# SensorsINI/v2e

Hardware: AMD Instinct MI355X
Metric: Mevents/s (EventEmulator.generate_events, 346x260, 10x slowdown) (higher is better)
Workload: dtype f64

## Files before the change

v2e_amd/csrc/emu.hip:

```cpp
#include "common.h"
#include "../../include/v2e_detmath.h"

#include <cstdarg>
#include <cstdlib>
#include <chrono>
#include <vector>

namespace {

constexpr int BLOCK = 256;
constexpr int WAVE = 64;
constexpr int RING = 64;
constexpr int SCAN_BLOCKS = 64;
constexpr int STAMP_LAUNCHES = 128;

constexpr uint32_t CNT_MASK = 0x00FFFFFFu;
constexpr uint32_t CNT_NEG = 1u << 24;
constexpr uint32_t CNT_SHOT_ON = 1u << 25;
constexpr uint32_t CNT_SHOT_OFF = 1u << 26;

struct FrameCtl {
    double t_prev, t_frame;
    double dt_over_tau;
    double shot_base;
// ... 1438 lines not shown
            V2E_HIP(hipHostGetDevicePointer((void **)&h->fr_ev_host_dev, h->fr_ev_host, 0));
            h->fr_ev_cap = want;
        }
        k_frame_rows_to_host<<<(unsigned)std::min<uint64_t>(v2e_cdiv((int64_t)n, 256), 4096), 256, 0, s>>>(
            (const float4 *)events_dev, rec, (float4 *)h->fr_ev_host_dev, nullptr, 0ull, n, nullptr);
        V2E_HIP(hipGetLastError());
        V2E_HIP(hipStreamSynchronize(s));
        *events_host = h->fr_ev_host;
        return 0;
    }
    if (user_rows) {
        if (n > est) {
            k_frame_rows_to_host<<<(unsigned)std::min<uint64_t>(v2e_cdiv((int64_t)(n - est), 256), 4096), 256, 0, s>>>(
                (const float4 *)events_dev, rec, (float4 *)user_rows_dev, nullptr, est, n - est, nullptr);
            V2E_HIP(hipGetLastError());
            V2E_HIP(hipStreamSynchronize(s));
        }
        if (n > 0) *events_host = user_rows;
        return 0;
    }
    if (n > est) {
        if (n > h->fr_ev_cap) {
            float *grown = nullptr;
            const uint64_t want = std::max<uint64_t>(2 * n, 1u << 16);
            V2E_HIP(hipHostMalloc((void **)&grown, sizeof(float) * 4 * want, hipHostMallocMapped));
            memcpy(grown, h->fr_ev_host, sizeof(float) * 4 * est);
            V2E_HIP(hipHostFree(h->fr_ev_host));
            h->fr_ev_host = grown; h->fr_ev_cap = want;
            V2E_HIP(hipHostGetDevicePointer((void **)&h->fr_ev_host_dev, h->fr_ev_host, 0));
        }
        k_frame_rows_to_host<<<(unsigned)std::min<uint64_t>(v2e_cdiv((int64_t)(n - est), 256), 4096), 256, 0, s>>>(
            (const float4 *)events_dev, rec, (float4 *)h->fr_ev_host_dev, nullptr, est, n - est, nullptr);
        V2E_HIP(hipGetLastError());
        V2E_HIP(hipStreamSynchronize(s));
    }
    if (n > 0) *events_host = h->fr_ev_host;
    return 0;
}

int v2e_emu_frame_host_rows(v2e_emu *h, float *pinned_rows, uint64_t cap_rows)
{
    V2E_REQUIRE(h, "null");
    h->fr_user_rows = h->fr_user_rows_dev = nullptr; h->fr_user_cap = 0;
    if (!pinned_rows || cap_rows == 0) return 0;
    V2E_HIP(hipSetDevice(h->device));
    void *dev = nullptr;
    V2E_HIP(hipHostGetDevicePointer(&dev, pinned_rows, 0));
    h->fr_user_rows = pinned_rows; h->fr_user_rows_dev = (float *)dev; h->fr_user_cap = cap_rows;
    return 0;
}

static int enqueue_run(v2e_emu *h, const v2e_emu_params *p, const KArgs &a, const void *frames, int dtype, int n_frames,
                       float *events, uint64_t cap, v2e_frame_rec *recs, hipStream_t s, hipEvent_t *evs = nullptr)
{
#define V2E_MARK(i) do { if (evs) V2E_HIP(hipEventRecord(evs[(i)], s)); } while (0)
    const RunScratch &r = h->cur();
    const size_t esz = dtype == V2E_DT_U8 ? 1 : (dtype == V2E_DT_F32 ? 4 : 8);
    V2E_HIP(zero_async(recs, sizeof(v2e_frame_rec) * (size_t)n_frames * h->n_clips, s));
    dim3 gridw(v2e_cdiv((int64_t)h->nwaves * WAVE, BLOCK), h->n_clips);
    for (int f = 0; f < n_frames; ++f) {
        const void *fr = (const char *)frames + (size_t)f * h->n_clips * h->npx * esz;
        const FrameCtl *ctl = r.run_ctl + (size_t)f * h->n_clips;
        v2e_frame_rec *rec = recs + (size_t)f * h->n_clips;
        const v2e_frame_rec *rec_prev = f > 0 ? rec - h->n_clips : nullptr;
        V2E_MARK(4 * f + 0);
        if (h->cs_sur) {
            dim3 gridp(v2e_cdiv(h->npx, BLOCK), h->n_clips);
            DISPATCH_FT(dtype, {
                if (p->f64_state) k_cs_lp<double, FT><<<gridp, BLOCK, 0, s>>>(a, (const FT *)fr, ctl, (double *)h->csr_lp);
                else k_cs_lp<float, FT><<<gridp, BLOCK, 0, s>>>(a, (const FT *)fr, ctl, (float *)h->csr_lp);
            });
            int rcs = v2e_csdvs_enqueue_frame(h->csr_lp, const_cast<void *>(h->cs_sur), h->csr_scratch, h->H, h->W, p->f64_state,
                                              h->csr_ap[f], h->csr_ah[f], h->csr_steps[f], h->csr_thr, h->csr_slots, h->csr_steps_dev + f, s);
            if (rcs) return rcs;
        }
        int rc = launch_count(h, a, p->f64_state, fr, dtype, ctl, r.run_fidx, (uint32_t)f, nullptr, nullptr, rec, s);
        if (rc) return rc;
        V2E_MARK(4 * f + 1);
        k_rank<<<gridw, BLOCK, 0, s>>>(a, ctl, rec, nullptr, 0);
        V2E_MARK(4 * f + 2);
        k_scan<<<dim3(SCAN_BLOCKS, h->n_clips), BLOCK, 0, s>>>(a, rec);
        V2E_MARK(4 * f + 3);
        if (p->f64_state) k_emit<double><<<gridw, BLOCK, 0, s>>>(a, ctl, rec, rec_prev, nullptr, r.run_fidx, (uint32_t)f, nullptr, 0, (float4 *)events, cap);
        else k_emit<float><<<gridw, BLOCK, 0, s>>>(a, ctl, rec, rec_prev, nullptr, r.run_fidx, (uint32_t)f, nullptr, 0, (float4 *)events, cap);
    }
    V2E_MARK(4 * n_frames);
#undef V2E_MARK
    V2E_HIP(hipGetLastError());
    return 0;
}


enum { ST_MAIN = 0, ST_AHEAD = 1, ST_SIDE = 2, ST_TAB = 3, ST_SIDE2 = 4, ST_COUNT = 5 };
enum { EV_FORK = 0, EV_JOIN = 1, EV_AHEAD = 2, EV_CHAIN = 3, EV_TAB = 4 };

struct Sched {
    v2e_emu *h;
    hipStream_t st[ST_COUNT];

    hipEvent_t real_event(int kind, int idx) const
    {
        switch (kind) {
        case EV_FORK: return h->ev_fork[idx];
        case EV_JOIN: return h->ev_join[idx];
        case EV_AHEAD: return h->ev_ahead[idx];
        case EV_CHAIN: return h->ev_chain[idx];
        default: return h->ev_tab[idx];
        }
    }
    int kernel(int s, const void *fn, dim3 grid, dim3 block, size_t lds, void **args)
    {
        V2E_HIP(hipLaunchKernel(fn, grid, block, args, lds, st[s]));
        return 0;
    }
    int zero4(int s, void *const ptr[4], const size_t bytes[4])
    {
        ZeroRanges z;
        unsigned long long tot = 0;
        for (int r = 0; r < 4; ++r) { z.p[r] = (uint32_t *)ptr[r]; z.n[r] = ptr[r] ? (bytes[r] + 3) / 4 : 0; tot += z.n[r]; }
        if (tot == 0) return 0;
        void *args[] = {(void *)&z};
        return kernel(s, (const void *)k_zero_ranges, dim3((unsigned)((tot + 255) / 256)), dim3(256), 0, args);
    }
    int record(int kind, int idx, int s)
    {
        V2E_HIP(hipEventRecord(real_event(kind, idx), st[s]));
        return 0;
    }
    int wait(int s, int kind, int idx)
    {
        V2E_HIP(hipStreamWaitEvent(st[s], real_event(kind, idx), 0));
        return 0;
    }
};

static int chain_egroups(const v2e_emu *h) { return (h->npx + GROUP_PX - 1) / GROUP_PX; }
static bool chain_small_grid(const v2e_emu *h) { return (long long)h->ngroups * h->n_clips <= 2ll * h->n_cu; }

static int chain_ring_batches(v2e_emu *h, bool pipelined)
{
    if (h->ch_ring_pref == 0) h->ch_ring_pref = (pipelined && chain_small_grid(h) && h->n_clips == 1) ? 5 : 3;
    return h->ch_ring_pref;
}

static bool chain_fused_records(const v2e_emu *h, int dtype, int nD)
{
    if (dtype != V2E_DT_U8) return true;
    if ((size_t)nD * 64 * h->n_clips * h->npx_pad * sizeof(uint2) >= (1ull << 32)) return true;
    const char *fe = getenv("V2E_AMD_CHAIN_FUSED");
    const int fused_env = fe ? atoi(fe) : -1;
    return fused_env >= 0 ? fused_env != 0 : !chain_small_grid(h);
}

static size_t chain_dyn_lds(bool fused) { return fused ? 0 : (size_t)CHAIN_SUB * BLOCK * sizeof(uint2); }

static const void *chain_fn(bool f64, int dtype, bool fused, bool allon = false)
{
    if (allon && f64 && dtype == V2E_DT_U8)
        return fused ? (const void *)k_chain<double, uint8_t, true, true> : (const void *)k_chain<double, uint8_t, false, true>;
    if (!fused) return f64 ? (const void *)k_chain<double, uint8_t, false> : (const void *)k_chain<float, uint8_t, false>;
    switch (dtype) {
    case V2E_DT_U8: return f64 ? (const void *)k_chain<double, uint8_t, true> : (const void *)k_chain<float, uint8_t, true>;
    case V2E_DT_F32: return f64 ? (const void *)k_chain<double, float, true> : (const void *)k_chain<float, float, true>;
    default: return f64 ? (const void *)k_chain<double, double, true> : (const void *)k_chain<float, double, true>;
    }
}

static int chain_blocks_per_cu(v2e_emu *h, bool f64, int dtype, bool fused, bool allon = false)
{
    allon = allon && f64 && dtype == V2E_DT_U8;
    const int key = (f64 ? 1 : 0) | ((dtype & 3) << 1) | (fused ? 8 : 0) | (allon ? 16 : 0);
    if (h->occ_cache[key] >= 0) return h->occ_cache[key];
    int per_cu = 0;
    if (hipOccupancyMaxActiveBlocksPerMultiprocessor(&per_cu, chain_fn(f64, dtype, fused, allon), BLOCK, chain_dyn_lds(fused)) != hipSuccess) per_cu = 0;
    if (per_cu > 2) per_cu = std::min(per_cu - 1, 6);
    h->occ_cache[key] = per_cu;
    return per_cu;
}

static int chain_frames_per_launch(const v2e_emu *h, bool has_refr, int flags, int max_blocks)
{
    int K = !has_refr ? CHAIN_K_MAX : (chain_small_grid(h) ? 32 : 8);
    if (const char *ev = getenv("V2E_AMD_CHAIN_K")) { const int v = atoi(ev); if (v >= 1 && v <= CHAIN_K_MAX) K = v; }
    if (has_refr && ((flags & V2E_RUN_ONE_FRAME_PER_LAUNCH) || h->ngroups > max_blocks)) K = 1;
    return K;
}

struct ChainLaunch { int f0, nf, pf0, pnf, wait_join, wait_ahead, ahead_next, emit_batch; };
static std::vector<ChainLaunch> chain_plan(int n_frames, int K, int E, int nD, bool has_refr, bool fused)
{
    const int m = E / K;
    const int nB = (n_frames + K - 1) / K;
    const int nL = has_refr ? nB + 1 : nB;
    const int nEB = (n_frames + E - 1) / E;
    std::vector<ChainLaunch> plan;
    for (int L = 0; L < nL; ++L) {
        ChainLaunch c;
        const bool tail = L >= nB;
        c.f0 = tail ? n_frames : L * K;
        c.nf = tail ? 0 : std::min((L + 1) * K, n_frames) - L * K;
        c.pf0 = (L - 1) * K;
        c.pnf = (has_refr && L > 0) ? std::min(L * K, n_frames) - (L - 1) * K : 0;
        const bool first = !tail && L % m == 0;
        c.wait_join = (first && L / m >= nD) ? L / m - nD : -1;
        c.wait_ahead = (first && !fused) ? L / m : -1;
        c.ahead_next = (first && !fused && L / m + 2 < nEB) ? L / m + 2 : -1;
        const int fin = has_refr ? L - 1 : L;
        c.emit_batch = (fin >= 0 && ((fin + 1) % m == 0 || fin == nB - 1)) ? fin / m : -1;
        plan.push_back(c);
    }
    return plan;
}

static bool emit_pull(size_t table_bytes)
{
    if (const char *e = getenv("V2E_AMD_EMIT_PULL")) { if (atoi(e) == 0) return false; }
    size_t budget = (size_t)24 << 30;
    if (const char *e = getenv("V2E_AMD_PULL_BUDGET_MB")) { const long long v = atoll(e); if (v >= 0) budget = (size_t)v << 20; }
    size_t free_b = 0, total_b = 0;
    if (hipMemGetInfo(&free_b, &total_b) != hipSuccess) return false;
    return table_bytes <= free_b / 4 && table_bytes <= budget;
}

static int chain_alloc(v2e_emu *h, const v2e_emu_params *p, int dtype, int n_frames, int flags, bool pipelined)
{
    const bool has_refr = p->refractory_period_s > 0;
    const int nD = chain_ring_batches(h, pipelined);
    const bool fused = chain_fused_records(h, dtype, nD);
    const int inst = (p->f64_state ? 1 : 0) | ((dtype & 3) << 1) | (fused ? 8 : 0);
    const bool allon_p = p->cutoff_hz > 0 && p->leak_rate_hz > 0 && p->shot_noise_rate_hz > 0 && has_refr;
    const int max_blocks = chain_blocks_per_cu(h, p->f64_state != 0, dtype, fused, allon_p) * h->n_cu;
    const int K = chain_frames_per_launch(h, has_refr, flags, max_blocks);
    int m = std::max(1, 64 / K);
    if (!chain_small_grid(h)) {
        if (h->ch_long_batches < 0) {
            size_t free_b = 0, total_b = 0;
            const size_t ring = (size_t)3 * 64 * h->n_clips * h->npx_pad * (sizeof(uint32_t) + sizeof(float) + sizeof(uint2));
            h->ch_long_batches = (hipMemGetInfo(&free_b, &total_b) == hipSuccess && ring <= free_b / 8) ? 1 : 0;
        }
        const int m_short = std::max(1, std::max(K, 8) / K);
        if (!h->ch_long_batches || (long long)m_short * K * h->n_clips >= 64) m = m_short;
    }
    if (const char *ev = getenv("V2E_AMD_CHAIN_M")) { const int v = atoi(ev); if (v >= 1 && v <= 64) m = v; }
    m = std::max(1, std::min(m, 64 / K));
    const int E = m * K;
    if (h->ch_K != K || h->ch_E != E || h->ch_nkeys_cap != h->nkeys_cap || h->ch_fused != (int)fused || h->ch_nD != nD) {
        h->sync_runs();
        h->free_chain_scratch();
        h->ch_launch_cap = 0;
        h->ch_K = K;
        h->ch_E = E;
        h->ch_fused = fused;
        h->ch_nD = nD;
        h->ch_D = nD * E;
        h->ch_nwp = (chain_egroups(h) + 15) / 16 * 16;
        h->ch_nkeys_cap = h->nkeys_cap;
        const size_t mask_bytes = 3 * sizeof(uint32_t) * 2 * GPX * E * (size_t)h->n_clips * h->nkeys_cap * h->ch_nwp;
        h->ch_pull = (h->ch_nwp / 16 <= 8192 && emit_pull(mask_bytes)) ? 1 : 0;
        h->drop_graphs();
    }
    const size_t nc = (size_t)h->n_clips;
    RunScratch &r = h->cur();
    if (!r.ch_cnt) {
        V2E_HIP(hipMalloc(&r.ch_cnt, sizeof(uint32_t) * h->ch_D * nc * h->npx_pad));
        V2E_HIP(hipMalloc(&r.ch_ruleM, sizeof(uint32_t) * h->ch_D * nc));
        V2E_HIP(hipMemset(r.ch_ruleM, 0, sizeof(uint32_t) * h->ch_D * nc));
        V2E_HIP(hipMalloc(&r.ch_wmax, 3 * sizeof(uint16_t) * E * nc * h->ch_nwp));
        V2E_HIP(hipMemset(r.ch_wmax, 0, 3 * sizeof(uint16_t) * E * nc * h->ch_nwp));
        V2E_HIP(hipMalloc(&r.ch_wtot, sizeof(uint16_t) * 3 * E * nc * h->nkeys_cap * h->ch_nwp));
        V2E_HIP(hipMemset(r.ch_wtot, 0, sizeof(uint16_t) * 3 * E * nc * h->nkeys_cap * h->ch_nwp));
        V2E_HIP(hipMalloc(&r.ch_cf, 3 * sizeof(CFrame) * E * nc));
        V2E_HIP(hipMemset(r.ch_cf, 0, 3 * sizeof(CFrame) * E * nc));
        V2E_HIP(hipMalloc(&r.ch_cdone, 3 * sizeof(unsigned) * E * nc));
        V2E_HIP(hipMemset(r.ch_cdone, 0, 3 * sizeof(unsigned) * E * nc));
        V2E_HIP(hipMalloc(&r.ch_cT, 3 * sizeof(uint32_t) * E * nc * h->nkeys_cap));
        V2E_HIP(hipMalloc(&r.ch_ckbase, 3 * sizeof(uint32_t) * E * nc * h->nkeys_cap));
        V2E_HIP(hipMalloc(&r.ch_cperm, 3 * sizeof(uint32_t) * E * nc * h->max_iters * 8));
        V2E_HIP(hipMalloc(&r.ch_cpre, 3 * sizeof(uint32_t) * E * nc * h->nkeys_cap * h->ch_nwp));
        if (h->ch_pull) {
            V2E_HIP(hipMalloc(&r.ch_cmask, 3 * sizeof(uint32_t) * 2 * GPX * E * nc * h->nkeys_cap * h->ch_nwp));
            V2E_HIP(hipMalloc(&r.ch_cpre16, 3 * sizeof(uint32_t) * E * nc * h->nkeys_cap * (h->ch_nwp / 16)));
        }
        if (!fused) {
            V2E_HIP(hipMalloc(&r.ch_rec, sizeof(uint2) * (size_t)h->ch_D * nc * h->npx_pad));
            V2E_HIP(hipMemset(r.ch_rec, 0, sizeof(uint2) * (size_t)h->ch_D * nc * h->npx_pad));
        }
        V2E_HIP(hipDeviceSynchronize());
        h->drop_graphs();
    }
    h->ch_max_blocks = max_blocks;
    h->ch_inst = inst;
    const int n_launch = (n_frames + K - 1) / K + 1;
    if (n_launch + 2 > h->run_off_cap) {
        h->sync_runs();
        for (RunScratch &q : h->sets) { hipFree(q.run_off); q.run_off = nullptr; }
        h->run_off_cap = n_launch + 2;
        h->drop_graphs();
    }
    if (!r.run_off) V2E_HIP(hipMalloc(&r.run_off, sizeof(unsigned long long) * (size_t)h->run_off_cap * h->n_clips));
    if (!h->ahead) V2E_HIP(hipStreamCreateWithFlags(&h->ahead, hipStreamNonBlocking));
    if (!h->tabs) V2E_HIP(hipStreamCreateWithFlags(&h->tabs, hipStreamNonBlocking));
    if (!h->side2) V2E_HIP(hipStreamCreateWithFlags(&h->side2, hipStreamNonBlocking));
    auto grow = [&](std::vector<hipEvent_t> &v, size_t n) -> int {
        while (v.size() < n) {
            hipEvent_t e;
            V2E_HIP(hipEventCreateWithFlags(&e, hipEventDisableTiming));
            v.push_back(e);
// ... 743 lines not shown
```

v2e_amd/csrc/emu_chain.h:

```cpp
#pragma once
#include "pull_index.h"

#ifndef V2E_CHAIN_LOCKSTEP
#define V2E_CHAIN_LOCKSTEP 0
#endif
#ifndef V2E_CHAIN_STAMPS
#define V2E_CHAIN_STAMPS 0
#endif

constexpr int CHAIN_K_MAX = 64;
constexpr int CFRAME_THREADS = 1024;
constexpr int CHAIN_SUB = 8;
constexpr int CHAIN_MAX_ITERS = 1024;

template <typename R> __device__ __forceinline__ R floor_div_pos(R a, R b)
{
    if (!(b > (R)0) || !(a >= (R)0)) return div_floor<R>(a, b);
    if (a < b) return (R)0;
    R q = floor(a / b);
    R r = fma(-q, b, a);
    if (r < (R)0) q -= (R)1;
    else if (r >= b) q += (R)1;
    return q;
}

__device__ __forceinline__ bool clip_barrier(unsigned *ctr, unsigned target, bool light = false)
{
    __shared__ int s_ok;
    asm volatile("s_waitcnt vmcnt(0)" ::: "memory");
    __syncthreads();
    if (threadIdx.x == 0) {
        if (!light) {
            __builtin_amdgcn_fence(__ATOMIC_RELEASE, "agent");
            asm volatile("s_waitcnt vmcnt(0)" ::: "memory");
        }
        __hip_atomic_fetch_add(ctr, 1u, __ATOMIC_RELAXED, __HIP_MEMORY_SCOPE_AGENT);
        unsigned spins = 0;
        int ok = 1;
        while (__hip_atomic_load(ctr, __ATOMIC_RELAXED, __HIP_MEMORY_SCOPE_AGENT) < target) {
            if (light) __builtin_amdgcn_s_sleep(1); else __builtin_amdgcn_s_sleep(4);
            if (++spins > 2000000u) { ok = 0; break; }
        }
        if (!light) __builtin_amdgcn_fence(__ATOMIC_ACQUIRE, "agent");
        s_ok = ok;
    }
    __syncthreads();
    return s_ok != 0;
}

struct FrameTab {
    float start, step, end;
    uint32_t refr_mask;
    __device__ __forceinline__ FrameTab(const FrameCtl *c, int lane)
        : start(c->ts_start[lane & 31]), step(c->ts_stepf[lane & 31]), end(c->ts_end), refr_mask(c->refr_mask) {}
};

__device__ __forceinline__ TsGen frame_tsgen(const KArgs &a, const FrameCtl *c, const FrameTab &ft, int n, bool &use_refr)
{
    if (n <= 32) {
        use_refr = a.has_refr && ((ft.refr_mask >> (n - 1)) & 1u);
        return TsGen(__uint_as_float(lane_value(__float_as_uint(ft.start), n - 1)), ft.end,
                     __uint_as_float(lane_value(__float_as_uint(ft.step), n - 1)), n);
    }
    const double t_prev = c->t_prev, t_frame = c->t_frame;
    use_refr = a.has_refr && a.refr > (t_frame - t_prev) / (double)n;
    FrameCtl cc;
    cc.t_prev = t_prev; cc.t_frame = t_frame;
    return TsGen(cc, n, nullptr);
}

typedef float v2e_f4 __attribute__((ext_vector_type(4)));
typedef unsigned int v2e_u4 __attribute__((ext_vector_type(4)));
typedef unsigned int v2e_u2 __attribute__((ext_vector_type(2)));

__device__ __forceinline__ double lane_value_d(double v, int idx)
{
    const unsigned long long u = (unsigned long long)__double_as_longlong(v);
    return __longlong_as_double((long long)(((unsigned long long)lane_value((uint32_t)(u >> 32), idx) << 32) | lane_value((uint32_t)u, idx)));
}
__device__ __forceinline__ void store_event_wt(float4 *ev_clip, unsigned long long row, float t, float x, float y, float pol)
{
    if (row < 0x7000000ull) {
        const __amdgpu_buffer_rsrc_t r = __builtin_amdgcn_make_buffer_rsrc((void *)ev_clip, 0, 0x7fffffff, 0x00020000);
        const v2e_f4 v = {t, x, y, pol};
        __builtin_amdgcn_raw_buffer_store_b128(v, r, (int)(row * 16ull), 0, 17);
    } else {
        ev_clip[row] = make_float4(t, x, y, pol);
    }
}

struct ChainArgs {
    const void *const *frames_pp;
    unsigned long long frame_stride;
    const uint32_t *fidx_base;
    const FrameCtl *ctl;
    int f0, nf;
    int pf0, pnf;
    int D, n_clips, K, ngroups;
    int slot_f0, slot_pf0;
    uint32_t *cnt;
    uint32_t *ruleM;
    float *tsold;
    const uint2 *rec;
    uint32_t *gM_prev, *gM_cur;
    unsigned *bar_prev;
    const void *base_in, *lp_in;
    const float *ts_in;
    void *base_out, *lp_out;
    float *ts_out;
    const void *base_pin, *lp_pin;
    const float *ts_pin;
    void *base_fix, *lp_fix;
    float *ts_fix;
    void *ckc_base, *ckc_lp;
    float *ckc_ts;
    void *ckp_base, *ckp_lp;
    float *ckp_ts;
    v2e_frame_rec *recs;
    int store_out;
    int prio;
    int bar_light;
    int lockstep;
    unsigned long long *dbg;
    unsigned long long *const *stamp_pp;
    int lidx;
};

#define WT_STORE(ptr, val) __hip_atomic_store((ptr), (val), __ATOMIC_RELAXED, __HIP_MEMORY_SCOPE_SYSTEM)

#define V2E_STAMP_C(i) do { if (V2E_CHAIN_STAMPS && ca.dbg && tid == 0) ca.dbg[(size_t)g * 16 + (i)] = wall_clock64(); } while (0)

template <typename FT>
__device__ __forceinline__ void frame_record_table(const KArgs &a, FT px, const float *s_lutL, const double *s_lutI, double dt_over_tau,
                                                   double &L, double &inten01, double &eps)
{
    constexpr bool U8 = sizeof(FT) == 1;
    if (U8) {
        L = a.log_input ? (double)px : (double)s_lutL[(int)px];
        inten01 = s_lutI[(int)px];
    } else {
        const double x = (double)px;
        L = a.log_input ? x : (double)lin_log(x);
        inten01 = a.use_inten ? (x + 20.0) / 275.0 : 0.0;
    }
    eps = 0.0;
    if (a.has_cutoff) {
        eps = inten01 * dt_over_tau;
        if (eps > 1.0) eps = 1.0;
    }
}

__device__ __forceinline__ void frame_record_rand(const KArgs &a, double inten01, double shot_base, float dtime_f, float lk, float thp,
                                                  float ppre, float npre, float rr, float uu, float &dl, uint32_t &sb)
{
    dl = 0.f;
    if (a.do_leak) {
        const float rate = lk * (1.0f - a.jit_f * rr);
        dl = (dtime_f * rate) * thp;
    }
    sb = 0;
    if (a.do_shot) {
        const double F = shot_base * (a.inten_slope * inten01 + 1);
        if ((double)uu > 1 - F * (double)ppre) sb |= 1u;
        if ((double)uu < F * (double)npre) sb |= 2u;
    }
}

__device__ __forceinline__ uint4 pack_frame_record(double eps, double L, uint32_t dl_bits, uint32_t sb)
{
    const unsigned long long eb = (unsigned long long)__double_as_longlong(eps);
    uint4 r;
    r.x = (uint32_t)eb;
    r.y = (uint32_t)(eb >> 32) | (sb << 30);
    r.z = __float_as_uint((float)L);
    r.w = dl_bits;
    return r;
}

template <typename FT>
__device__ __forceinline__ uint4 make_frame_record(const KArgs &a, FT px, const float *s_lutL, const double *s_lutI, double dt_over_tau,
                                                   double shot_base, float dtime_f, float lk, float thp, float ppre, float npre, float rr,
                                                   float uu)
{
    double L, inten01, eps;
    frame_record_table<FT>(a, px, s_lutL, s_lutI, dt_over_tau, L, inten01, eps);
    float dl;
    uint32_t sb;
    frame_record_rand(a, inten01, shot_base, dtime_f, lk, thp, ppre, npre, rr, uu, dl, sb);
    return pack_frame_record(eps, L, __float_as_uint(dl), sb);
}

__device__ __forceinline__ uint4 decode_frame_record(const KArgs &a, uint2 r8, const float *s_lutL, const double *s_lutI, double dt_over_tau)
{
    double L, inten01, eps;
    frame_record_table<uint8_t>(a, (uint8_t)(r8.y & 0xFFu), s_lutL, s_lutI, dt_over_tau, L, inten01, eps);
    return pack_frame_record(eps, L, r8.x, r8.y >> 30);
}

struct AheadArgs {
    const void *const *frames_pp;
    unsigned long long frame_stride;
    const FrameCtl *ctl;
    const uint32_t *fidx_base;
    int f0, nf, D, n_clips;
    int slot0;
    int ppt;
    uint2 *rec;
};

template <typename FT>
__global__ __launch_bounds__(BLOCK) void k_ahead(KArgs a, AheadArgs aa)
{
    static_assert(sizeof(FT) == 1, "k_ahead's records carry the pixel byte: uint8 frames only");
    __shared__ double s_lutI[256];
    const int tid = threadIdx.x;
    s_lutI[tid] = a.lut_I[tid];
    __syncthreads();
    const int clip = blockIdx.y, p = blockIdx.x * BLOCK + tid;
    if (p >= a.npx) return;
    const uint32_t fbase = *aa.fidx_base;
    const char *const frames = (const char *)*aa.frames_pp;
    const size_t sp = (size_t)clip * a.npx_pad + p;
    const bool need_r = a.do_leak && a.jit_f != 0.f;
    const float thp = a.pos_thres[sp], thn = a.neg_thres[sp];
    const float lk = a.do_leak ? a.leak_hz_f * a.noise_rate[sp] : 0.f;
    const float ppre = a.scalar_thres ? a.pos_pre_scalar : a.pos_nom_f / thp;
    const float npre = a.scalar_thres ? a.neg_pre_scalar : a.neg_nom_f / thn;
    v2e_philox_keys ks;
    v2e_philox_key_schedule((uint32_t)a.seed, (uint32_t)(a.seed >> 32), &ks);
    for (int zz = 0; zz < aa.ppt; ++zz) {
        const uint32_t q = v2e_frame_pair(fbase + (uint32_t)aa.f0) + blockIdx.z * (uint32_t)aa.ppt + (uint32_t)zz;
        const int f_odd = (int)(2u * q - 1u - fbase);
        const bool in0 = f_odd >= aa.f0 && f_odd < aa.f0 + aa.nf, in1 = f_odd + 1 >= aa.f0 && f_odd + 1 < aa.f0 + aa.nf;
        if (!in0 && !in1) continue;
        float r_odd = 0.f, u_odd = 0.f, r_even = 0.f, u_even = 0.f;
        if (need_r || a.do_shot) v2e_draw_pair_ks(&ks, (uint32_t)clip, q, (uint32_t)p, need_r, &r_odd, &u_odd, &r_even, &u_even);
#pragma unroll
        for (int half = 0; half < 2; ++half) {
            if (!(half ? in1 : in0)) continue;
            const int f = f_odd + half;
            int sl = aa.slot0 + (f - aa.f0);
            if (sl >= aa.D) sl -= aa.D;
            const FrameCtl *c = aa.ctl + (f * aa.n_clips + clip);
            const FT px = ((const FT *)(frames + (size_t)f * aa.frame_stride))[(size_t)clip * a.npx + p];
            float dl;
            uint32_t sb;
            frame_record_rand(a, s_lutI[px], c->shot_base, (float)(c->t_frame - c->t_prev), lk, thp, ppre, npre, half ? r_even : r_odd,
                              half ? u_even : u_odd, dl, sb);
            aa.rec[((uint32_t)sl * (uint32_t)aa.n_clips + (uint32_t)clip) * (uint32_t)a.npx_pad + (uint32_t)p] =
                make_uint2(__float_as_uint(dl), (uint32_t)px | (sb << 30));
        }
    }
}

template <typename R> __device__ __forceinline__ R floor_div_rcp(R a, R b, R rb)
{
    R q = floor(a * rb);
    R r = fma(-q, b, a);
    const bool lo = r < (R)0, hi = r >= b;
    q = lo ? q - (R)1 : (hi ? q + (R)1 : q);
    r = lo ? r + b : (hi ? r - b : r);
    if (__builtin_expect(!(r >= (R)0 && r < b), 0)) return floor_div_pos<R>(a, b);
    return q;
}

template <typename R, typename FT, bool FUSED, bool ALLON = false>
__global__ __launch_bounds__(BLOCK)
__attribute__((amdgpu_waves_per_eu((FUSED && sizeof(R) == 8 && sizeof(FT) == 1) ? 5 : 1, 8)))
void k_chain(KArgs a_in, ChainArgs ca)
{
    KArgs a = a_in;
    if (ALLON) { a.has_cutoff = 1; a.do_leak = 1; a.do_shot = 1; a.has_refr = 1; a.use_inten = 1; }
    extern __shared__ uint2 s_arec[];
    __shared__ float s_lutL[256];
    __shared__ double s_lutI[256];
    __shared__ double s_dtau[FUSED ? CHAIN_K_MAX : 1], s_shot[FUSED ? CHAIN_K_MAX : 1];
    __shared__ float s_dtime[FUSED ? CHAIN_K_MAX : 1];
    constexpr bool U8 = sizeof(FT) == 1;
    const int tid = threadIdx.x, lane = tid & (WAVE - 1);
    const int g = blockIdx.x;
    const int p = g * BLOCK + tid;
    const bool valid = p < a.npx;
    if (ca.prio) __builtin_amdgcn_s_setprio(3);
    V2E_STAMP_C(0);
    unsigned long long *const stamp = *ca.stamp_pp;
    if (stamp && tid == 0) atomicMax(stamp + 2 * ca.lidx, ~wall_clock64());
    uint32_t fbase = 0u;
    const char *frames = nullptr;
    float tab_L = 0.f;
    double tab_I = 0.0;
    if (!FUSED) {
        tab_L = a.lut_L[tid];
        tab_I = a.lut_I[tid];
    }
    if (FUSED) {
        fbase = *ca.fidx_base;
        frames = (const char *)*ca.frames_pp;
        if (U8) {
            s_lutL[tid] = a.lut_L[tid];
            s_lutI[tid] = a.lut_I[tid];
        }
    }
    const bool need_r = a.do_leak && a.jit_f != 0.f;

    for (int clip = blockIdx.y; clip < ca.n_clips; clip += (int)gridDim.y) {
        if (clip != (int)blockIdx.y) __syncthreads();
        const size_t sp = (size_t)clip * a.npx_pad + p;
        auto wrap_slot = [&](const int sl) __attribute__((always_inline)) -> int { return sl >= ca.D ? sl - ca.D : sl; };
        const uint32_t lane_px = (uint32_t)((size_t)clip * a.npx_pad + p);
        const uint32_t slot_px = (uint32_t)((size_t)ca.n_clips * a.npx_pad);
        const __amdgpu_buffer_rsrc_t rec_rsrc = __builtin_amdgcn_make_buffer_rsrc((void *)ca.rec, 0, -1, 0x00020000);
        const __amdgpu_buffer_rsrc_t cnt_rsrc = __builtin_amdgcn_make_buffer_rsrc((void *)ca.cnt, 0, -1, 0x00020000);
        auto load_rec = [&](const int sl) __attribute__((always_inline)) -> uint2 {
            const v2e_u2 v = __builtin_amdgcn_raw_buffer_load_b64(rec_rsrc, (int)(lane_px * 8u), (int)((uint32_t)sl * slot_px * 8u), 0);
            return make_uint2(v.x, v.y);
        };
        auto decode_rec = [&](const uint2 r8, const double dtau_v, const int k) __attribute__((always_inline)) -> uint4 {
            const double dtau = a.has_cutoff ? lane_value_d(dtau_v, k) : 0.0;
            const uint4 r = decode_frame_record(a, r8, s_lutL, s_lutI, dtau);
            return valid ? r : make_uint4(0u, 0u, 0u, 0u);
        };
        auto stage = [&](const int sl0, const int fn) __attribute__((always_inline)) {
            if (FUSED) return;
            uint2 t[CHAIN_SUB];
            int sl = sl0;
#pragma unroll
            for (int j = 0; j < CHAIN_SUB; ++j) {
                t[j] = make_uint2(0u, 0u);
                if (j < fn && valid) t[j] = load_rec(sl);
                if (++sl == ca.D) sl = 0;
            }
#pragma unroll
            for (int j = 0; j < CHAIN_SUB; ++j)
                if (j < fn) s_arec[(size_t)j * BLOCK + tid] = t[j];
        };
        auto fill_scalars = [&](const int fs, const int fn) __attribute__((always_inline)) {
            if (!FUSED) return;
            __syncthreads();
            if (tid < fn) {
                const FrameCtl *c = ca.ctl + (size_t)(fs + tid) * ca.n_clips + clip;
                s_dtau[tid] = c->dt_over_tau;
                s_shot[tid] = c->shot_base;
                s_dtime[tid] = (float)(c->t_frame - c->t_prev);
            }
            __syncthreads();
        };
        float thp = 1.f, thn = 1.f;
        R b = (R)0, lp = (R)0;
        float tsm = 0.f;
        const bool lp_state = a.has_cutoff || a.do_shot || ca.store_out;
        if (valid) {
            thp = a.pos_thres[sp];
            thn = a.neg_thres[sp];
            b = ((const R *)ca.base_in)[sp];
            if (lp_state) lp = ((const R *)ca.lp_in)[sp];
            if (a.has_refr) tsm = ca.ts_in[sp];
        }
        bool own = !(a.has_refr && ca.pnf > 0);
        uint32_t gM_v = 0u;
        if (!own && lane < ca.pnf) gM_v = ca.gM_prev[(size_t)clip * ca.K + lane];
        uint32_t mon_own = 0xFFFFFFFFu, mon_prev = 0xFFFFFFFFu;
        if (a.has_refr) {
            if (lane < ca.nf) mon_own = ca.ctl[(size_t)(ca.f0 + lane) * ca.n_clips + clip].refr_on_n;
            if (!own && lane < ca.pnf) mon_prev = ca.ctl[(size_t)(ca.pf0 + lane) * ca.n_clips + clip].refr_on_n;
        }
        double dtau_own = 0.0, dtau_prev = 0.0;
        if (!FUSED && a.has_cutoff) {
            if (lane < ca.nf) dtau_own = ca.ctl[(size_t)(ca.f0 + lane) * ca.n_clips + clip].dt_over_tau;
            if (!own && lane < ca.pnf) dtau_prev = ca.ctl[(size_t)(ca.pf0 + lane) * ca.n_clips + clip].dt_over_tau;
        }
        double dtau_r = 0.0, shot_r = 0.0;
        float dtime_r = 0.f, nr = 0.f;
        if (FUSED && tid < ca.nf) {
            const FrameCtl *c = ca.ctl + (size_t)(ca.f0 + tid) * ca.n_clips + clip;
            dtau_r = c->dt_over_tau;
            shot_r = c->shot_base;
            dtime_r = (float)(c->t_frame - c->t_prev);
        }
        if (FUSED && valid && a.do_leak) nr = a.noise_rate[sp];
        stage(ca.slot_f0, ca.nf);
        if (FUSED)
            asm volatile("s_waitcnt vmcnt(0)" : "+v"(b), "+v"(lp), "+v"(tsm), "+v"(thp), "+v"(thn), "+v"(gM_v), "+v"(mon_own), "+v"(mon_prev) : : "memory");
        else
            asm volatile("s_waitcnt vmcnt(0)" : "+v"(b), "+v"(lp), "+v"(tsm), "+v"(thp), "+v"(thn), "+v"(gM_v), "+v"(mon_own), "+v"(mon_prev),
                         "+v"(dtau_own), "+v"(dtau_prev), "+v"(tab_L), "+v"(tab_I) : : "memory");
        if (!FUSED && clip == (int)blockIdx.y) {
            s_lutL[tid] = tab_L;
            s_lutI[tid] = tab_I;
            __syncthreads();
        }
        if (FUSED) {
            if (tid < CHAIN_K_MAX) {
                s_dtau[tid] = dtau_r;
                s_shot[tid] = shot_r;
                s_dtime[tid] = dtime_r;
            }
            __syncthreads();
        }
        const float lk = a.leak_hz_f * nr;
        const float ppre = a.scalar_thres ? a.pos_pre_scalar : a.pos_nom_f / thp;
        const float npre = a.scalar_thres ? a.neg_pre_scalar : a.neg_nom_f / thn;
        const R tpd = a.scalar_thres ? (R)a.pos_div : (R)thp;
        const R tnd = a.scalar_thres ? (R)a.neg_div : (R)thn;
        R rtp = (R)1 / tpd, rtn = (R)1 / tnd;
        asm volatile("" : "+v"(rtp), "+v"(rtn));
        V2E_STAMP_C(1);
        bool redone = false;
        int round = 0, last_exact = -1;
        uint32_t pred_v = 0u;
        uint32_t exact_v = 0u;
        int c0 = 0;
        int bar_idx = 0;
        int lock_k = -1;
        for (;;) {
            int fs, fn;
            uint32_t *gM_dst;
            if (!own) {
                if (round > 0) {
                    gM_v = 0u;
                    if (lane < ca.pnf) gM_v = __hip_atomic_load(ca.gM_prev + ((size_t)round * ca.n_clips + clip) * ca.K + lane, __ATOMIC_RELAXED, __HIP_MEMORY_SCOPE_AGENT);
                }
                const unsigned long long hit = __ballot(gM_v != pred_v && lane > last_exact);
                const int j = hit ? (int)__builtin_ctzll(hit) : -1;
                if (j < 0) {
                    own = true;
                } else {
                    if (lane > last_exact) exact_v = gM_v;
                    pred_v = lane > j ? gM_v : 0u;
                    last_exact = j;
                    ++round;
                    redone = true;
                    lock_k = (V2E_CHAIN_LOCKSTEP && ca.lockstep && __builtin_amdgcn_readlane((int)gM_v, j) != 0 && j + 1 < ca.pnf) ? j + 1 : -1;
                    c0 = ca.ckp_base ? (j / CHAIN_SUB) * CHAIN_SUB : 0;
                    if (valid) {
                        if (c0 == 0) {
                            b = ((const R *)ca.base_pin)[sp];
                            if (lp_state) lp = ((const R *)ca.lp_pin)[sp];
                            tsm = ca.ts_pin[sp];
                        } else {
                            const size_t cs = ((size_t)(c0 / CHAIN_SUB - 1) * ca.n_clips + clip) * a.npx_pad + p;
                            b = ((const R *)ca.ckp_base)[cs];
                            if (lp_state) lp = ((const R *)ca.ckp_lp)[cs];
                            tsm = ca.ckp_ts[cs];
                        }
                    }
                    asm volatile("s_waitcnt vmcnt(0)" : "+v"(b), "+v"(lp), "+v"(tsm) : : "memory");
                }
            }
            if (own) { fs = ca.f0; fn = ca.nf; gM_dst = ca.gM_cur + (size_t)clip * ca.K; c0 = 0; }
            else { fs = ca.pf0; fn = ca.pnf; gM_dst = ca.gM_prev + ((size_t)round * ca.n_clips + clip) * ca.K; }
            const int fs_slot = own ? ca.slot_f0 : ca.slot_pf0;
            const double dtau_v = own ? dtau_own : dtau_prev;
            if (redone) {
                fill_scalars(fs, fn);
                stage(wrap_slot(fs_slot + c0), fn - c0);
            }
            const uint32_t mon_v = own ? mon_own : mon_prev;
            void *const ck_base = own ? ca.ckc_base : ca.ckp_base;
            void *const ck_lp = own ? ca.ckc_lp : ca.ckp_lp;
            float *const ck_ts = own ? ca.ckc_ts : ca.ckp_ts;
            if (own) V2E_STAMP_C(2);
            float r_odd = 0.f, u_odd = 0.f, r_even = 0.f, u_even = 0.f;
            bool have_pair = false;
            uint32_t rule_v = 0u;
            const bool thr_bad = !(tpd > (R)0) || !(tnd > (R)0);
            constexpr double QMAX = sizeof(R) == 8 ? 1.0e9 : 1.0e6;
            auto frame_body = [&](const int k, const int js) __attribute__((always_inline)) -> uint32_t {
                const int f = fs + k;
                const uint32_t Mon = (uint32_t)__builtin_amdgcn_readlane((int)mon_v, k);
                uint32_t exM = own ? 0u : (uint32_t)__builtin_amdgcn_readlane((int)exact_v, k);
                uint4 rc = make_uint4(0u, 0u, 0u, 0u);
                if (FUSED) {
                    FT px = (FT)0;
                    if (valid) px = ((const FT *)(frames + (size_t)f * ca.frame_stride))[(size_t)clip * a.npx + p];
                    const uint32_t gf = fbase + (uint32_t)f;
                    if (need_r || a.do_shot) {
                        if (!have_pair || v2e_frame_half(gf) == 0u)
                            v2e_draw_pair(a.seed, (uint32_t)clip, v2e_frame_pair(gf), (uint32_t)p, need_r, &r_odd, &u_odd, &r_even, &u_even);
                        have_pair = true;
                    }
                    const bool even = v2e_frame_half(gf) != 0u;
                    rc = make_frame_record<FT>(a, px, s_lutL, s_lutI, s_dtau[k], s_shot[k], s_dtime[k], lk, thp, ppre, npre,
                                               even ? r_even : r_odd, even ? u_even : u_odd);
                } else {
                    rc = decode_rec(s_arec[(size_t)js * BLOCK + tid], dtau_v, k);
                }
                const double eps = __longlong_as_double((long long)(((unsigned long long)(rc.y & 0x3FFFFFFFu) << 32) | rc.x));
                const double L = (double)__uint_as_float(rc.z);
                R lpn;
                if (a.has_cutoff) lpn = (R)((1.0 - eps) * (double)lp + eps * L);
                else lpn = (R)L;
                if (a.do_leak) b = b - (R)__uint_as_float(rc.w);
                const R diff = (lpn + (R)0.0f) - b;
                const bool is_pos = diff > (R)0;
                const bool neg = !is_pos;
                const R bt = is_pos ? tpd : tnd, rbt = is_pos ? rtp : rtn;
                const R am = sizeof(R) == 8 ? (R)__builtin_fabs((double)diff) : (R)__builtin_fabsf((float)diff);
                const R q0 = floor(am * rbt);
                const R r0 = fma(-q0, bt, am);
                int mag = (int)q0;
                mag -= (r0 < (R)0) ? 1 : 0;
                mag += (r0 >= bt) ? 1 : 0;
                asm volatile("" : "+v"(mag));
                if (__builtin_expect(!(q0 <= (R)QMAX) || thr_bad, 0)) {
                    const R mg = is_pos ? diff : ((-diff) > (R)0 ? -diff : (R)0);
                    const int q = (int)floor_div_pos<R>(mg, bt);
                    mag = q > 0 ? q : 0;
                }
                if (FUSED && !valid) mag = 0;
                uint32_t cw = ((uint32_t)mag & CNT_MASK) | ((mag > 0 && neg) ? CNT_NEG : 0u);
                if (a.do_shot) cw |= (rc.y >> 5) & (CNT_SHOT_ON | CNT_SHOT_OFF);
                if (FUSED && !valid) cw = 0u;
                if (FUSED) {
                    if (valid) WT_STORE(&ca.cnt[((size_t)wrap_slot(fs_slot + k) * ca.n_clips + clip) * a.npx_pad + p], cw);
                }
                const int magv = mag;
                if (a.has_refr && k > (own ? -1 : last_exact) && __ballot((uint32_t)magv >= Mon) != 0ull) {
                    const int wm = wave_max_i32(magv);
                    if (lane == 0) atomicMax(gM_dst + k, (uint32_t)wm);
                }
                if (V2E_CHAIN_LOCKSTEP && !own && k == lock_k) {
                    __builtin_amdgcn_s_setprio(0);
                    const bool okb = clip_barrier(ca.bar_prev + (size_t)bar_idx * ca.n_clips + clip, (unsigned)ca.ngroups, ca.bar_light != 0);
                    ++bar_idx;
                    if (ca.prio) __builtin_amdgcn_s_setprio(3);
                    if (!okb && tid == 0) atomicOr(&ca.recs[(size_t)ca.pf0 * ca.n_clips + clip].flags, V2E_FLAG_SYNC_TIMEOUT);
                    uint32_t mk = 0u;
                    if (lane == 0) mk = __hip_atomic_load(gM_dst + k, __ATOMIC_RELAXED, __HIP_MEMORY_SCOPE_AGENT);
                    mk = (uint32_t)__builtin_amdgcn_readfirstlane((int)mk);
                    exM = mk;
                    if (lane == k) { exact_v = mk; pred_v = mk; }
                    last_exact = k;
                    lock_k = (mk != 0u && k + 1 < fn) ? k + 1 : -1;
                }
                int fcount = magv;
                if (exM != 0u) {
                    const FrameCtl *c = ca.ctl + (size_t)f * ca.n_clips + clip;
                    const FrameTab ftb(c, lane);
                    bool ruled = false;
                    const TsGen tg = frame_tsgen(a, c, ftb, (int)exM, ruled);
                    if (ruled) {
                        if (lane == k) rule_v = exM;
                        if (valid) ca.tsold[((size_t)wrap_slot(fs_slot + k) * ca.n_clips + clip) * a.npx_pad + p] = tsm;
                        fcount = 0;
                        const int nit = min(magv, 1 << 16);
                        for (int i = 0; i < nit; ++i) {
                            const float t = tg(i);
                            const float pt = 1.0f * t - tsm;
                            if (pt > a.refr_f) { tsm = t; ++fcount; }
                        }
                    }
                }
                {
                    float d = (float)fcount * (neg ? thn : thp);
                    d = neg ? -d : d;
                    const R bn = b + (R)d;
                    const bool shot = a.do_shot && (rc.y >> 30) != 0u;
                    b = shot ? lpn : bn;
                }
                lp = lpn;
                if (V2E_CHAIN_STAMPS && own && k < 12) V2E_STAMP_C(3 + k);
                return cw;
            };
            uint2 nx[CHAIN_SUB];
            auto fetch_next = [&](const int kn) __attribute__((always_inline)) {
                const int cn = min(CHAIN_SUB, fn - kn);
                int sl = cn > 0 ? wrap_slot(fs_slot + kn) : 0;
#pragma unroll
                for (int j = 0; j < CHAIN_SUB; ++j) {
                    nx[j] = make_uint2(0u, 0u);
                    if (!FUSED && valid && j < cn) nx[j] = load_rec(sl);
                    if (++sl == ca.D) sl = 0;
                }
            };
            fetch_next(c0 + CHAIN_SUB);
            for (int k0 = c0; k0 < fn; k0 += CHAIN_SUB) {
                if (ck_base && k0 > c0 && valid) {
                    const size_t cs = ((size_t)(k0 / CHAIN_SUB - 1) * ca.n_clips + clip) * a.npx_pad + p;
                    ((R *)ck_base)[cs] = b;
                    if (lp_state) ((R *)ck_lp)[cs] = lp;
                    ck_ts[cs] = tsm;
                }
                __builtin_amdgcn_sched_barrier(0);
                const int kend = min(k0 + CHAIN_SUB, fn);
                const int slot0 = wrap_slot(fs_slot + k0);
                uint32_t cwq[CHAIN_SUB];
#pragma unroll
                for (int j = 0; j < CHAIN_SUB; ++j) cwq[j] = 0u;
                if (kend - k0 == CHAIN_SUB) {
#pragma unroll
                    for (int j = 0; j < CHAIN_SUB; ++j) cwq[j] = frame_body(k0 + j, j);
                } else {
#pragma unroll
                    for (int j = 0; j < CHAIN_SUB; ++j)
                        if (k0 + j < kend) cwq[j] = frame_body(k0 + j, j);
                }
                if (!FUSED) {
                    const int rem = fn - k0 - CHAIN_SUB;
                    const int nnext = min(CHAIN_SUB, rem);
#pragma unroll
                    for (int j = 0; j < CHAIN_SUB; ++j)
                        if (j < nnext) s_arec[(size_t)j * BLOCK + tid] = nx[j];
                    fetch_next(k0 + 2 * CHAIN_SUB);
                    if (valid) {
                        int sl = slot0;
#pragma unroll
                        for (int j = 0; j < CHAIN_SUB; ++j) {
                            if (k0 + j < kend)
                                __builtin_amdgcn_raw_buffer_store_b32(cwq[j], cnt_rsrc, (int)(lane_px * 4u), (int)((uint32_t)sl * slot_px * 4u), 17);
                            if (++sl == ca.D) sl = 0;
                        }
                    }
                }
            }
            if (a.has_refr && g == 0 && tid < WAVE) {
                int sl = fs_slot + lane;
                if (sl >= ca.D) sl -= ca.D;
                if (lane >= c0 && lane < fn) WT_STORE(&ca.ruleM[(size_t)sl * ca.n_clips + clip], rule_v);
            }
            if (own) break;
            if (valid) {
                ((R *)ca.base_fix)[sp] = b;
                if (lp_state) ((R *)ca.lp_fix)[sp] = lp;
                ca.ts_fix[sp] = tsm;
            }
            if (last_exact >= ca.pnf - 1) continue;
            __builtin_amdgcn_s_setprio(0);
            const bool ok = clip_barrier(ca.bar_prev + (size_t)bar_idx * ca.n_clips + clip, (unsigned)ca.ngroups, ca.bar_light != 0);
            ++bar_idx;
            if (ca.prio) __builtin_amdgcn_s_setprio(3);
            if (!ok && tid == 0) atomicOr(&ca.recs[(size_t)ca.pf0 * ca.n_clips + clip].flags, V2E_FLAG_SYNC_TIMEOUT);
        }
        if (valid && (ca.nf > 0 || ca.store_out || redone)) {
            ((R *)ca.base_out)[sp] = b;
            if (ca.nf > 0 || lp_state) ((R *)ca.lp_out)[sp] = lp;
            if (a.has_refr) ca.ts_out[sp] = tsm;
        }
        V2E_STAMP_C(15);
    }
    if (stamp && tid == 0) atomicMax(stamp + 2 * ca.lidx + 1, wall_clock64());
}

struct CFrame {
    int M;
    uint32_t n_events, n_signal, discarded;
};

struct CEmitArgs {
    const FrameCtl *ctl;
    v2e_frame_rec *recs;
    const uint32_t *fidx_base;
    int f0, nE, D, n_clips, nwp, nwaves, E;
    int slot0;
    const uint32_t *cnt;
    const uint32_t *ruleM;
    uint16_t *wmax;
    uint16_t *wtot;
    const float *tsold;
    CFrame *cf;
    uint32_t *cT;
    uint32_t *ckbase;
    uint32_t *cperm;
    uint32_t *cpre;
    float4 *events;
    unsigned long long cap;
    const unsigned long long *off_in;
    unsigned long long *off_out;
    unsigned *cdone;
    int capw, ich;
    int zpw_tot, zpw_emit;
    int coff_in_cemit;
    uint32_t *cmask;
    int wpf, p2;
    uint32_t *cpre16;
};

#ifndef V2E_GPX
#define V2E_GPX 4
#endif
constexpr int GPX = V2E_GPX;
constexpr int GROUP_PX = GPX * WAVE;
constexpr int GROUP_SRC_BITS = GPX <= 4 ? 8 : (GPX <= 8 ? 9 : 10);

constexpr int CTOT_ZF = 2;

__global__ __launch_bounds__(BLOCK) void k_ctot(KArgs a, CEmitArgs ea)
{
    const int tid = threadIdx.x, lane = tid & (WAVE - 1), wave = tid / WAVE;
    const int clip = blockIdx.y;
    const int grp = blockIdx.x * (BLOCK / WAVE) + wave;
    if (grp >= ea.nwaves) return;
    const int p0 = grp * GROUP_PX + lane;
    const int zb = (int)blockIdx.z * CTOT_ZF;
    uint32_t cwq[CTOT_ZF][GPX], rMq[CTOT_ZF];
    int slotq[CTOT_ZF];
    {
        int sl = ea.slot0 + zb;
        if (sl >= ea.D) sl -= ea.D;
#pragma unroll
        for (int q = 0; q < CTOT_ZF; ++q) {
            slotq[q] = sl;
            rMq[q] = 0u;
#pragma unroll
            for (int j = 0; j < GPX; ++j) {
                cwq[q][j] = 0u;
                if (zb + q < ea.nE && p0 + j * WAVE < a.npx) cwq[q][j] = ea.cnt[((size_t)sl * ea.n_clips + clip) * a.npx_pad + p0 + j * WAVE];
            }
            if (zb + q < ea.nE && ea.ruleM) rMq[q] = ea.ruleM[(size_t)sl * ea.n_clips + clip];
            if (++sl == ea.D) sl = 0;
        }
    }
#pragma unroll
    for (int q = 0; q < CTOT_ZF; ++q) {
        const int z = zb + q;
        if (z >= ea.nE) break;
        const size_t zc = (size_t)z * ea.n_clips + clip;
        const uint32_t rM = (uint32_t)__builtin_amdgcn_readfirstlane((int)rMq[q]);
        int magv[GPX];
        bool neg[GPX];
        unsigned long long negb[GPX];
        int mmax = 0;
        uint32_t son = 0, soff = 0;
        unsigned long long sob[GPX], sfb[GPX];
#pragma unroll
        for (int j = 0; j < GPX; ++j) {
            const uint32_t cw = cwq[q][j];
            magv[j] = (int)(cw & CNT_MASK);
            neg[j] = (cw & CNT_NEG) != 0;
            negb[j] = __ballot(neg[j]);
            mmax = max(mmax, magv[j]);
            sob[j] = __ballot((cw & CNT_SHOT_ON) != 0);
            sfb[j] = __ballot((cw & CNT_SHOT_OFF) != 0);
            son += (uint32_t)__popcll(sob[j]);
            soff += (uint32_t)__popcll(sfb[j]);
        }
        const int wm = wave_max_i32(mmax);
        if (lane == 0) ea.wmax[zc * ea.nwp + grp] = (uint16_t)min(wm, 65535);
        uint16_t *trow = ea.wtot + (zc * a.nkeys_cap) * ea.nwp + grp;
        uint32_t *mrow = ea.cmask ? ea.cmask + ((zc * a.nkeys_cap + (lane >= 2 * GPX ? 1 : 0)) * ea.nwp + grp) * (2 * GPX) + (lane & (2 * GPX - 1)) : nullptr;
        auto put_masks = [&](const int key_on, const unsigned long long (&on_m)[GPX], const unsigned long long (&off_m)[GPX]) __attribute__((always_inline)) {
            uint32_t mw = 0u;
#pragma unroll
            for (int j = 0; j < GPX; ++j) {
                asm("v_writelane_b32 %0, %1, %2" : "+v"(mw) : "s"((uint32_t)on_m[j]), "n"(2 * j));
                asm("v_writelane_b32 %0, %1, %2" : "+v"(mw) : "s"((uint32_t)(on_m[j] >> 32)), "n"(2 * j + 1));
                asm("v_writelane_b32 %0, %1, %2" : "+v"(mw) : "s"((uint32_t)off_m[j]), "n"(2 * GPX + 2 * j));
                asm("v_writelane_b32 %0, %1, %2" : "+v"(mw) : "s"((uint32_t)(off_m[j] >> 32)), "n"(2 * GPX + 2 * j + 1));
            }
            if (lane < 4 * GPX) mrow[(size_t)key_on * ea.nwp * (2 * GPX)] = mw;
        };
        static_assert(4 * GPX == 16, "k_ctot: the mask words of an iteration are one 16-lane DPP row");
        uint32_t pmask = 0u;
        if (mrow) {
#pragma unroll
            for (int j = 0; j < GPX; ++j) {
// ... 724 lines not shown
```

Measured before the change: 19270.

## Keep chain records in registers, pre-decode sub-batches, and add light frame path

In the non-fused chain kernel, prefetched records now stay in registers and are decoded one sub-batch ahead into per-frame coefficients (1-eps, eps*L, leak, shot bits), so the LDS staging buffer is removed. When no lane in a sub-batch needs exact refractory replay, a light variant of the frame body skips the per-frame readlanes and ballots and batches the refractory max checks after the sub-batch. The kernel's waves-per-eu lower bound is raised for non-fused variants. The change trades more register pressure, which may cost occupancy or cause spills, for less LDS traffic and fewer cross-lane operations on the serial chain.

```diff
diff --git a/v2e_amd/csrc/emu.hip b/v2e_amd/csrc/emu.hip
--- a/v2e_amd/csrc/emu.hip
+++ b/v2e_amd/csrc/emu.hip
@@ -1614,7 +1614,7 @@
     return fused_env >= 0 ? fused_env != 0 : !chain_small_grid(h);
 }
 
-static size_t chain_dyn_lds(bool fused) { return fused ? 0 : (size_t)CHAIN_SUB * BLOCK * sizeof(uint2); }
+static size_t chain_dyn_lds(bool) { return 0; }
 
 static const void *chain_fn(bool f64, int dtype, bool fused, bool allon = false)
 {
diff --git a/v2e_amd/csrc/emu_chain.h b/v2e_amd/csrc/emu_chain.h
--- a/v2e_amd/csrc/emu_chain.h
+++ b/v2e_amd/csrc/emu_chain.h
@@ -1,4 +1,5 @@
 #pragma once
+#include <type_traits>
 #include "pull_index.h"
 
 #ifndef V2E_CHAIN_LOCKSTEP
@@ -192,8 +193,15 @@
 
 __device__ __forceinline__ uint4 decode_frame_record(const KArgs &a, uint2 r8, const float *s_lutL, const double *s_lutI, double dt_over_tau)
 {
-    double L, inten01, eps;
-    frame_record_table<uint8_t>(a, (uint8_t)(r8.y & 0xFFu), s_lutL, s_lutI, dt_over_tau, L, inten01, eps);
+    const int px = (int)(r8.y & 0xFFu);
+    const float tl = s_lutL[px];
+    const double inten01 = s_lutI[px];
+    const double L = a.log_input ? (double)px : (double)tl;
+    double eps = 0.0;
+    if (a.has_cutoff) {
+        eps = inten01 * dt_over_tau;
+        if (eps > 1.0) eps = 1.0;
+    }
     return pack_frame_record(eps, L, r8.x, r8.y >> 30);
 }
 
@@ -266,12 +274,11 @@
 
 template <typename R, typename FT, bool FUSED, bool ALLON = false>
 __global__ __launch_bounds__(BLOCK)
-__attribute__((amdgpu_waves_per_eu((FUSED && sizeof(R) == 8 && sizeof(FT) == 1) ? 5 : 1, 8)))
+__attribute__((amdgpu_waves_per_eu((FUSED && sizeof(R) == 8 && sizeof(FT) == 1) ? 5 : (FUSED ? 1 : 2), 8)))
 void k_chain(KArgs a_in, ChainArgs ca)
 {
     KArgs a = a_in;
     if (ALLON) { a.has_cutoff = 1; a.do_leak = 1; a.do_shot = 1; a.has_refr = 1; a.use_inten = 1; }
-    extern __shared__ uint2 s_arec[];
     __shared__ float s_lutL[256];
     __shared__ double s_lutI[256];
     __shared__ double s_dtau[FUSED ? CHAIN_K_MAX : 1], s_shot[FUSED ? CHAIN_K_MAX : 1];
@@ -320,19 +327,32 @@
             const uint4 r = decode_frame_record(a, r8, s_lutL, s_lutI, dtau);
             return valid ? r : make_uint4(0u, 0u, 0u, 0u);
         };
+        uint2 st[CHAIN_SUB];
         auto stage = [&](const int sl0, const int fn) __attribute__((always_inline)) {
             if (FUSED) return;
-            uint2 t[CHAIN_SUB];
             int sl = sl0;
 #pragma unroll
             for (int j = 0; j < CHAIN_SUB; ++j) {
-                t[j] = make_uint2(0u, 0u);
-                if (j < fn && valid) t[j] = load_rec(sl);
+                st[j] = make_uint2(0u, 0u);
+                if (j < fn && valid) st[j] = load_rec(sl);
                 if (++sl == ca.D) sl = 0;
             }
-#pragma unroll
-            for (int j = 0; j < CHAIN_SUB; ++j)
-                if (j < fn) s_arec[(size_t)j * BLOCK + tid] = t[j];
+        };
+        double dq_om[CHAIN_SUB], dq_el[CHAIN_SUB];
+        float dq_dl[CHAIN_SUB];
+        uint32_t dq_sb[CHAIN_SUB];
+        auto decode_sub = [&](const uint2 *r, const int kb, const double dtau_v) __attribute__((always_inline)) {
+            if (FUSED) return;
+#pragma unroll
+            for (int j = 0; j < CHAIN_SUB; ++j) {
+                const uint4 rc = decode_rec(r[j], dtau_v, (kb + j) & (WAVE - 1));
+                const double eps = __longlong_as_double((long long)(((unsigned long long)(rc.y & 0x3FFFFFFFu) << 32) | rc.x));
+                const double L = (double)__uint_as_float(rc.z);
+                dq_om[j] = 1.0 - eps;
+                dq_el[j] = a.has_cutoff ? eps * L : L;
+                dq_dl[j] = __uint_as_float(rc.w);
+                dq_sb[j] = (rc.y >> 5) & (CNT_SHOT_ON | CNT_SHOT_OFF);
+            }
         };
         auto fill_scalars = [&](const int fs, const int fn) __attribute__((always_inline)) {
             if (!FUSED) return;
@@ -465,10 +485,11 @@
             uint32_t rule_v = 0u;
             const bool thr_bad = !(tpd > (R)0) || !(tnd > (R)0);
             constexpr double QMAX = sizeof(R) == 8 ? 1.0e9 : 1.0e6;
-            auto frame_body = [&](const int k, const int js) __attribute__((always_inline)) -> uint32_t {
+            auto frame_body = [&](auto light_c, const int k, const int js, uint32_t &magq) __attribute__((always_inline)) -> uint32_t {
+                constexpr bool LIGHT = decltype(light_c)::value;
                 const int f = fs + k;
-                const uint32_t Mon = (uint32_t)__builtin_amdgcn_readlane((int)mon_v, k);
-                uint32_t exM = own ? 0u : (uint32_t)__builtin_amdgcn_readlane((int)exact_v, k);
+                const uint32_t Mon = LIGHT ? 0u : (uint32_t)__builtin_amdgcn_readlane((int)mon_v, k);
+                uint32_t exM = (LIGHT || own) ? 0u : (uint32_t)__builtin_amdgcn_readlane((int)exact_v, k);
                 uint4 rc = make_uint4(0u, 0u, 0u, 0u);
                 if (FUSED) {
                     FT px = (FT)0;
@@ -482,15 +503,24 @@
                     const bool even = v2e_frame_half(gf) != 0u;
                     rc = make_frame_record<FT>(a, px, s_lutL, s_lutI, s_dtau[k], s_shot[k], s_dtime[k], lk, thp, ppre, npre,
                                                even ? r_even : r_odd, even ? u_even : u_odd);
+                }
+                R lpn;
+                float dl;
+                uint32_t sbw;
+                if (FUSED) {
+                    const double eps = __longlong_as_double((long long)(((unsigned long long)(rc.y & 0x3FFFFFFFu) << 32) | rc.x));
+                    const double L = (double)__uint_as_float(rc.z);
+                    if (a.has_cutoff) lpn = (R)((1.0 - eps) * (double)lp + eps * L);
+                    else lpn = (R)L;
+                    dl = __uint_as_float(rc.w);
+                    sbw = (rc.y >> 5) & (CNT_SHOT_ON | CNT_SHOT_OFF);
                 } else {
-                    rc = decode_rec(s_arec[(size_t)js * BLOCK + tid], dtau_v, k);
-                }
-                const double eps = __longlong_as_double((long long)(((unsigned long long)(rc.y & 0x3FFFFFFFu) << 32) | rc.x));
-                const double L = (double)__uint_as_float(rc.z);
-                R lpn;
-                if (a.has_cutoff) lpn = (R)((1.0 - eps) * (double)lp + eps * L);
-                else lpn = (R)L;
-                if (a.do_leak) b = b - (R)__uint_as_float(rc.w);
+                    if (a.has_cutoff) lpn = (R)(dq_om[js] * (double)lp + dq_el[js]);
+                    else lpn = (R)dq_el[js];
+                    dl = dq_dl[js];
+                    sbw = dq_sb[js];
+                }
+                if (a.do_leak) b = b - (R)dl;
                 const R diff = (lpn + (R)0.0f) - b;
                 const bool is_pos = diff > (R)0;
                 const bool neg = !is_pos;
@@ -509,17 +539,18 @@
                 }
                 if (FUSED && !valid) mag = 0;
                 uint32_t cw = ((uint32_t)mag & CNT_MASK) | ((mag > 0 && neg) ? CNT_NEG : 0u);
-                if (a.do_shot) cw |= (rc.y >> 5) & (CNT_SHOT_ON | CNT_SHOT_OFF);
+                if (a.do_shot) cw |= sbw;
                 if (FUSED && !valid) cw = 0u;
                 if (FUSED) {
                     if (valid) WT_STORE(&ca.cnt[((size_t)wrap_slot(fs_slot + k) * ca.n_clips + clip) * a.npx_pad + p], cw);
                 }
                 const int magv = mag;
-                if (a.has_refr && k > (own ? -1 : last_exact) && __ballot((uint32_t)magv >= Mon) != 0ull) {
+                magq = (uint32_t)magv;
+                if (!LIGHT && a.has_refr && k > (own ? -1 : last_exact) && __ballot((uint32_t)magv >= Mon) != 0ull) {
                     const int wm = wave_max_i32(magv);
                     if (lane == 0) atomicMax(gM_dst + k, (uint32_t)wm);
                 }
-                if (V2E_CHAIN_LOCKSTEP && !own && k == lock_k) {
+                if (V2E_CHAIN_LOCKSTEP && !LIGHT && !own && k == lock_k) {
                     __builtin_amdgcn_s_setprio(0);
                     const bool okb = clip_barrier(ca.bar_prev + (size_t)bar_idx * ca.n_clips + clip, (unsigned)ca.ngroups, ca.bar_light != 0);
                     ++bar_idx;
@@ -534,7 +565,7 @@
                     lock_k = (mk != 0u && k + 1 < fn) ? k + 1 : -1;
                 }
                 int fcount = magv;
-                if (exM != 0u) {
+                if (!LIGHT && exM != 0u) {
                     const FrameCtl *c = ca.ctl + (size_t)f * ca.n_clips + clip;
                     const FrameTab ftb(c, lane);
                     bool ruled = false;
@@ -555,7 +586,7 @@
                     float d = (float)fcount * (neg ? thn : thp);
                     d = neg ? -d : d;
                     const R bn = b + (R)d;
-                    const bool shot = a.do_shot && (rc.y >> 30) != 0u;
+                    const bool shot = a.do_shot && sbw != 0u;
                     b = shot ? lpn : bn;
                 }
                 lp = lpn;
@@ -573,6 +604,7 @@
                     if (++sl == ca.D) sl = 0;
                 }
             };
+            decode_sub(st, c0, dtau_v);
             fetch_next(c0 + CHAIN_SUB);
             for (int k0 = c0; k0 < fn; k0 += CHAIN_SUB) {
                 if (ck_base && k0 > c0 && valid) {
@@ -584,23 +616,45 @@
                 __builtin_amdgcn_sched_barrier(0);
                 const int kend = min(k0 + CHAIN_SUB, fn);
                 const int slot0 = wrap_slot(fs_slot + k0);
-                uint32_t cwq[CHAIN_SUB];
-#pragma unroll
-                for (int j = 0; j < CHAIN_SUB; ++j) cwq[j] = 0u;
-                if (kend - k0 == CHAIN_SUB) {
-#pragma unroll
-                    for (int j = 0; j < CHAIN_SUB; ++j) cwq[j] = frame_body(k0 + j, j);
+                uint32_t cwq[CHAIN_SUB], magq[CHAIN_SUB];
+#pragma unroll
+                for (int j = 0; j < CHAIN_SUB; ++j) cwq[j] = magq[j] = 0u;
+                const bool light = !FUSED && (own || (!V2E_CHAIN_LOCKSTEP && ((__ballot(exact_v != 0u) >> k0) & 0xFFull) == 0ull));
+                if (light && kend - k0 == CHAIN_SUB) {
+#pragma unroll
+                    for (int j = 0; j < CHAIN_SUB; ++j) cwq[j] = frame_body(std::true_type{}, k0 + j, j, magq[j]);
+                } else if (light) {
+#pragma unroll
+                    for (int j = 0; j < CHAIN_SUB; ++j)
+                        if (k0 + j < kend) cwq[j] = frame_body(std::true_type{}, k0 + j, j, magq[j]);
+                } else if (kend - k0 == CHAIN_SUB) {
+#pragma unroll
+                    for (int j = 0; j < CHAIN_SUB; ++j) cwq[j] = frame_body(std::false_type{}, k0 + j, j, magq[j]);
                 } else {
 #pragma unroll
                     for (int j = 0; j < CHAIN_SUB; ++j)
-                        if (k0 + j < kend) cwq[j] = frame_body(k0 + j, j);
+                        if (k0 + j < kend) cwq[j] = frame_body(std::false_type{}, k0 + j, j, magq[j]);
                 }
                 if (!FUSED) {
                     const int rem = fn - k0 - CHAIN_SUB;
-                    const int nnext = min(CHAIN_SUB, rem);
-#pragma unroll
-                    for (int j = 0; j < CHAIN_SUB; ++j)
-                        if (j < nnext) s_arec[(size_t)j * BLOCK + tid] = nx[j];
+                    if (rem > 0) decode_sub(nx, k0 + CHAIN_SUB, dtau_v);
+                    if (light && a.has_refr) {
+                        unsigned long long hit[CHAIN_SUB], any = 0ull;
+#pragma unroll
+                        for (int j = 0; j < CHAIN_SUB; ++j) {
+                            const uint32_t Mon = (uint32_t)__builtin_amdgcn_readlane((int)mon_v, (k0 + j) & (WAVE - 1));
+                            hit[j] = (k0 + j < kend && k0 + j > (own ? -1 : last_exact)) ? __ballot(magq[j] >= Mon) : 0ull;
+                            any |= hit[j];
+                        }
+                        if (__builtin_expect(any != 0ull, 0)) {
+#pragma unroll
+                            for (int j = 0; j < CHAIN_SUB; ++j)
+                                if (hit[j] != 0ull) {
+                                    const int wm = wave_max_i32((int)magq[j]);
+                                    if (lane == 0) atomicMax(gM_dst + k0 + j, (uint32_t)wm);
+                                }
+                        }
+                    }
                     fetch_next(k0 + 2 * CHAIN_SUB);
                     if (valid) {
                         int sl = slot0;
```

After: 20110, median of 6. +4.3%, better.
